# CMU-Perceptual-Computing-Lab/caffe_rtpose

Measured on AMD Instinct MI355X. Metric: frames/sec (whole node) at 656x368 COCO model, higher is better.
Workload: dtype f16; 1 GPU; COCO 656x368, 1 scale(s), synthetic 720p video: pageable host u8 1280x720 frames through rtp_submit_frame: pinned copy + H2D + device warp / INTER_AREA / normalise / pad inside the timed region -> conv stack+ImResize+NMS+connect -> joints on the host; precision mode mixed, 7 frames in flight/GPU in ; precision=mixed, input=host_u8, batch_frames=2, frames_in_flight=7, num_scales=1, exec=graph, hw_queues=4, parallelism=frame-sharded replicas x1

## Files before the change

### caffe_rtpose_amd/csrc/conv_pw2.hip

```cpp
#include "conv_common.h"
#include <atomic>
#include <type_traits>

namespace rtp {

namespace {
constexpr int PW_BM = 64;
constexpr int PW_ROW = 256;
constexpr int PW_STR = PW_ROW + 16;
constexpr int PW_X = PW_BM * PW_STR;
constexpr int PW_W = 128 * PW_STR;
constexpr int PW_MAXMID = 512;
constexpr int PW_LDS = 4 * PW_X + PW_W + PW_MAXMID * 4;
static_assert(PW_LDS >= 64 * 64 * 4, "epilogue scratch fits");
}

typedef unsigned int u32x32 __attribute__((ext_vector_type(32)));
typedef unsigned int u32x16 __attribute__((ext_vector_type(16)));
template <typename V>
__device__ __forceinline__ void pw_fetch(V& reg, const unsigned char* src, int tid) {
  constexpr int NV = sizeof(V) / 16;
#pragma unroll
  for (int i = 0; i < NV; ++i) {
    const uint4 t = *(const uint4*)(src + (size_t)(tid + i * 256) * 16);
    reg[4 * i] = t.x; reg[4 * i + 1] = t.y; reg[4 * i + 2] = t.z; reg[4 * i + 3] = t.w;
  }
}
template <typename V>
__device__ __forceinline__ void pw_stash(const V& reg, unsigned char* sW, int tid) {
  constexpr int NV = sizeof(V) / 16;
#pragma unroll
  for (int i = 0; i < NV; ++i) {
    const int v = tid + i * 256;
    uint4 t;
    t.x = reg[4 * i]; t.y = reg[4 * i + 1]; t.z = reg[4 * i + 2]; t.w = reg[4 * i + 3];
    *(uint4*)(sW + (v >> 4) * PW_STR + (v & 15) * 16) = t;
  }
}

__global__ __launch_bounds__(256) void conv_pw2_kernel(Pw2Params Q) {
  const KStamp kstamp_(Q.P2.stamp);
  extern __shared__ __attribute__((aligned(16))) unsigned char smem[];
  unsigned char* sXh = smem;
  unsigned char* sXl = smem + PW_X;
  unsigned char* sHh = smem + 2 * PW_X;
  unsigned char* sHl = smem + 3 * PW_X;
  unsigned char* sW = smem + 4 * PW_X;
  float* sB1 = (float*)(smem + 4 * PW_X + PW_W);

  const ConvParams& P = Q.P2;
  const int tid = threadIdx.x, lane = tid & 63, wave = tid >> 6;
  const int lrow = lane & 31, lhalf = lane >> 5;
  const int total_m = P.tiles_per_img * P.nimg;
  const int prob = blockIdx.x / total_m;
  const int mt = blockIdx.x % total_m;
  const int img = mt / P.tiles_per_img;
  const int m0 = (mt % P.tiles_per_img) * PW_BM;
  const ConvProblem& pr = P.prob[prob];
  const long pix0 = (long)img * P.img_pix + (long)P.halo * P.Wp + m0;
  const int Mtot = P.H * P.Wp;
  int stamp_i = 0;
  auto stamp = [&]() __attribute__((always_inline)) {
    if (P.clkprobe && blockIdx.x == 0 && tid == 0 && stamp_i < 31) P.clkprobe[1 + stamp_i++] = wall_clock64();
  };
  stamp();

  const float* b1p = prob ? Q.b1[1] : Q.b1[0];
  const int nmid = Q.c1_chunks * 128;
  const float b_a = tid < nmid ? b1p[tid] : 0.f;
  const float b_b = tid + 256 < nmid ? b1p[tid + 256] : 0.f;
  u32x16 r_xh, r_xl;
  {
    const _Float16* xin = (const _Float16*)(prob ? Q.x_in[1] : Q.x_in[0]) + pix0 * Q.x_cstride;
#pragma unroll
    for (int i = 0; i < 4; ++i) {
      const int v = tid + i * 256, row = v >> 4, seg = v & 15;
      const unsigned char* src = (const unsigned char*)(xin + (long)row * Q.x_cstride) + seg * 16;
      const uint4 h = *(const uint4*)src;
      r_xh[4 * i] = h.x; r_xh[4 * i + 1] = h.y; r_xh[4 * i + 2] = h.z; r_xh[4 * i + 3] = h.w;
      if (Q.x_lo_off) {
        const uint4 l = *(const uint4*)(src + (size_t)Q.x_lo_off * 2);
        r_xl[4 * i] = l.x; r_xl[4 * i + 1] = l.y; r_xl[4 * i + 2] = l.z; r_xl[4 * i + 3] = l.w;
      }
    }
  }
  u32x32 r_w1h, r_w1l;
  u32x16 r_w2h, r_w2l;
  auto lds_barrier = [&]() __attribute__((always_inline)) { asm volatile("s_waitcnt lgkmcnt(0)\n\ts_barrier" ::: "memory"); };
  auto gemm = [&](const unsigned char* a_img, int a_row0, auto ntm_tag, int b_row0, floatx16* acc) __attribute__((always_inline)) {
    constexpr int NT = decltype(ntm_tag)::value;
    const unsigned char* pb = sW + (b_row0 + lrow) * PW_STR + lhalf * 16;
    const unsigned char* pa = a_img + (a_row0 + lrow) * PW_STR + lhalf * 16;
#pragma unroll
    for (int g = 0; g < 8; ++g) {
      const uint4 fb = *(const uint4*)(pb + g * 32);
#pragma unroll
      for (int i = 0; i < NT; ++i) {
        const uint4 fa = *(const uint4*)(pa + i * 32 * PW_STR + g * 32);
        Mma<_Float16>::run(fa, fb, acc[i]);
      }
    }
  };
  const std::integral_constant<int, 2> two{};
  const std::integral_constant<int, 1> one{};

  const int w1_parts = Q.split_w1 ? 2 : 1, w2_parts = Q.split_w2 ? 2 : 1;
  const unsigned char* w1 = (const unsigned char*)(prob ? Q.w1[1] : Q.w1[0]);
  const unsigned char* w2 = (const unsigned char*)(prob ? P.prob[1].w : P.prob[0].w);
  const size_t W1_BLK = 128 * PW_ROW, W2_BLK = 64 * PW_ROW;
  auto w1_blk = [&](int c, int part) { return w1 + ((size_t)c * w1_parts + part) * W1_BLK; };
  auto w2_blk = [&](int c, int part) { return w2 + ((size_t)c * w2_parts + part) * W2_BLK; };

  floatx16 acc2;
#pragma unroll
  for (int q = 0; q < 16; ++q) acc2[q] = 0.f;

  pw_fetch(r_w1h, w1_blk(0, 0), tid);
  if (Q.split_w1) pw_fetch(r_w1l, w1_blk(0, 1), tid);
  pw_fetch(r_w2h, w2_blk(0, 0), tid);
  if (Q.split_w2) pw_fetch(r_w2l, w2_blk(0, 1), tid);
  sB1[tid] = b_a;
  sB1[tid + 256] = b_b;
#pragma unroll
  for (int i = 0; i < 4; ++i) {
    const int v = tid + i * 256, row = v >> 4, seg = v & 15;
    uint4 t;
    t.x = r_xh[4 * i]; t.y = r_xh[4 * i + 1]; t.z = r_xh[4 * i + 2]; t.w = r_xh[4 * i + 3];
    *(uint4*)(sXh + row * PW_STR + seg * 16) = t;
    if (Q.x_lo_off) {
      t.x = r_xl[4 * i]; t.y = r_xl[4 * i + 1]; t.z = r_xl[4 * i + 2]; t.w = r_xl[4 * i + 3];
      *(uint4*)(sXl + row * PW_STR + seg * 16) = t;
    }
  }
  stamp();
  for (int c = 0; c < Q.c1_chunks; ++c) {
    const bool more = c + 1 < Q.c1_chunks;
    floatx16 acc1[2];
#pragma unroll
    for (int i = 0; i < 2; ++i)
#pragma unroll
      for (int q = 0; q < 16; ++q) acc1[i][q] = 0.f;
    lds_barrier();
    pw_stash(r_w1h, sW, tid);
    if (more) pw_fetch(r_w1h, w1_blk(c + 1, 0), tid);
    lds_barrier();
    stamp();
    gemm(sXh, 0, two, wave * 32, acc1);
    if (Q.x_lo_off) gemm(sXl, 0, two, wave * 32, acc1);
    stamp();
    if (Q.split_w1) {
      lds_barrier();
      pw_stash(r_w1l, sW, tid);
      if (more) pw_fetch(r_w1l, w1_blk(c + 1, 1), tid);
      lds_barrier();
      gemm(sXh, 0, two, wave * 32, acc1);
      stamp();
    }
    {
      const float bias = sB1[c * 128 + wave * 32 + lrow];
#pragma unroll
      for (int i = 0; i < 2; ++i)
#pragma unroll
        for (int q = 0; q < 16; ++q) {
          const int row = i * 32 + (q & 3) + 8 * (q >> 2) + 4 * lhalf;
          float v = acc1[i][q] + bias;
          if (Q.relu1) v = v > 0.f ? v : 0.f;
          const _Float16 hi = (_Float16)v;
          *(_Float16*)(sHh + row * PW_STR + (wave * 32 + lrow) * 2) = hi;
          if (Q.h_lo) *(_Float16*)(sHl + row * PW_STR + (wave * 32 + lrow) * 2) = (_Float16)(v - (float)hi);
        }
    }
    stamp();
    lds_barrier();
    pw_stash(r_w2h, sW, tid);
    if (more) pw_fetch(r_w2h, w2_blk(c + 1, 0), tid);
    lds_barrier();
    stamp();
    gemm(sHh, (wave >> 1) * 32, one, (wave & 1) * 32, &acc2);
    if (Q.h_lo) gemm(sHl, (wave >> 1) * 32, one, (wave & 1) * 32, &acc2);
    stamp();
    const ConvDst& md = prob ? Q.mid[1] : Q.mid[0];
    if (md.base) {
      for (int v = tid; v < PW_BM * 16; v += 256) {
        const int row = v >> 4, seg = v & 15;
        const int m = m0 + row;
        const int xp = m - (m / P.Wp) * P.Wp;
        if (m >= Mtot || xp < P.halo || xp >= P.halo + P.W) continue;
        _Float16* dp = (_Float16*)md.base + (pix0 + row) * md.cstride + md.coff + c * 128 + seg * 8;
        *(uint4*)dp = *(const uint4*)(sHh + row * PW_STR + seg * 16);
        if (md.lo_off) *(uint4*)(dp + md.lo_off) = *(const uint4*)(sHl + row * PW_STR + seg * 16);
      }
    }
    stamp();
    if (Q.split_w2) {
      lds_barrier();
      pw_stash(r_w2l, sW, tid);
      if (more) pw_fetch(r_w2l, w2_blk(c + 1, 1), tid);
      lds_barrier();
      gemm(sHh, (wave >> 1) * 32, one, (wave & 1) * 32, &acc2);
      stamp();
    }
  }
  __syncthreads();
  stamp();
  floatx16 acc[1][1] = {{acc2}};
  conv_epilogue<_Float16, 64, 64, 2, 2, 1, 1, 1>(P, pr, acc, smem, 0, wave, (wave >> 1) * 32, (wave & 1) * 32, lane, img, m0, 0);
  stamp();
  if (P.clkprobe && blockIdx.x == 0 && tid == 0) P.clkprobe[0] = stamp_i;
}

hipError_t launch_conv_pw2(const Pw2Params& Q, int nprob, int nimg, hipStream_t stream) {
  static std::atomic<unsigned> attr_mask{0};
  int dev = 0;
  (void)hipGetDevice(&dev);
  if (!(attr_mask.load(std::memory_order_relaxed) & (1u << (dev & 31)))) {
    hipError_t e = hipFuncSetAttribute((const void*)conv_pw2_kernel, hipFuncAttributeMaxDynamicSharedMemorySize, PW_LDS);
    if (e != hipSuccess) return e;
    attr_mask.fetch_or(1u << (dev & 31), std::memory_order_relaxed);
  }
  dim3 grid(Q.P2.tiles_per_img * nimg * nprob);
  hipLaunchKernelGGL(conv_pw2_kernel, grid, dim3(256), PW_LDS, stream, Q);
  return hipGetLastError();
}

}
```

### caffe_rtpose_amd/csrc/engine.cpp

```cpp
#include <hip/hip_runtime.h>

#include <algorithm>
#include <atomic>
#include <chrono>
#include <cmath>
#include <cstdarg>
#include <cstdio>
#include <cstring>
#include <deque>
#include <fstream>
#include <map>
#include <mutex>
#include <sstream>
#include <string>
#include <thread>
#include <vector>

#include "../../include/rtpose_mi355x.h"
#include "kernels.h"
#include "netdef.h"
#include "plan.h"

using namespace rtp;

// ... 195 lines not shown
  }
  const int M = (int)std::nearbyint(std::ldexp(a, 9));
  return (unsigned char)(sign | (unsigned)(M == 8 ? 8 : M));
}

template <typename T>
void pack_conv(const Plan& plan, const ConvOp& c, const std::vector<float>& w, const std::vector<float>& b,
               std::vector<unsigned char>* out_w, std::vector<float>* out_b) {
  const Tensor& ti = plan.tensors[c.in_tensor];
  const int per_chunk = c.rowb / (int)sizeof(T);
  const int taps = c.k_eff * c.k_eff;
  out_w->assign(c.w_bytes, 0);
  T* pw = (T*)out_w->data();
  auto kpos = [&](int n, int kk) {
    if (c.impl == 0) return kk;
    const int per16 = 16 / (int)sizeof(T);
    const int c16 = kk / per16, within = kk % per16;
    return ((c16 ^ conv_ring_swz(c.rowb, n)) * per16) + within;
  };
  if (c.direct_first) {
    for (int t = 0; t < 2; ++t)
      for (int j = 0; j < 2; ++j)
        for (int l = 0; l < 64; ++l) {
          const int n = t * 32 + conv_first_channel_of_row(l & 31);
          for (int e2 = 0; e2 < 8; ++e2) {
            const int k = j * 16 + (l >> 5) * 8 + e2;
            float wv = 0.f;
            if (k < 27) { const int r = k / 9, s2 = (k % 9) / 3, cc = k % 3; wv = w[((size_t)(n * 3 + cc) * 3 + r) * 3 + s2]; }
            pw[((size_t)(t * 2 + j) * 64 + l) * 8 + e2] = (T)wv;
          }
        }
    out_b->assign(c.CoutP, 0.f);
    for (int n = 0; n < c.cout; ++n) (*out_b)[n] = b[n];
    return;
  }
  if (c.fused) {
    const int rows = c.fused == 1 ? 128 : 64;
    const int parts = c.split_w ? 2 : 1;
    for (int n = 0; n < c.cout; ++n)
      for (int cr = 0; cr < c.cin; ++cr) {
        const int ci = ti.chmap[cr];
        const int chunk = c.fused == 1 ? n / 128 : ci / 128;
        const int row = c.fused == 1 ? n % 128 : n;
        const int k = ci % 128;
        const float wv = w[(size_t)n * c.cin + cr];
        const T hi = (T)wv;
        pw[(((size_t)chunk * parts + 0) * rows + row) * 128 + k] = hi;
        if (c.split_w) pw[(((size_t)chunk * parts + 1) * rows + row) * 128 + k] = (T)(wv - (float)hi);
      }
    out_b->assign(c.CoutP, 0.f);
    for (int n = 0; n < c.cout; ++n) (*out_b)[n] = b[n];
    return;
  }
  if (c.first) {
    for (int n = 0; n < c.cout; ++n)
      for (int r = 0; r < 3; ++r)
        for (int s = 0; s < 3; ++s)
          for (int cc = 0; cc < 3; ++cc) {
            const int j = (r * 3 + s) * 3 + cc;
            const int chunk = j / per_chunk, kk = j % per_chunk;
            const float wv = w[((size_t)(n * 3 + cc) * 3 + r) * 3 + s];
            const T hi = (T)wv;
            pw[((size_t)(0 * c.nchunk + chunk) * c.CoutP + n) * per_chunk + kpos(n, kk)] = hi;
            if (c.split_w) pw[((size_t)(0 * c.nchunk + c.ncp + chunk) * c.CoutP + n) * per_chunk + kpos(n, kk)] = (T)(wv - (float)hi);
          }
  } else {
    for (int n = 0; n < c.cout; ++n)
      for (int cr = 0; cr < c.cin; ++cr) {
        const int ci = ti.chmap[cr];
        const int chunk = ci / per_chunk, kk = ci % per_chunk;
        for (int r = 0; r < c.k; ++r)
          for (int s = 0; s < c.k; ++s) {
            const int tap = r * c.k + s;
            const float wv = w[((size_t)(n * c.cin + cr) * c.k + r) * c.k + s];
            const T hi = (T)wv;
            const T lo = (T)(wv - (float)hi);
            if (c.h8) {
              const size_t tile0 = (size_t)(r * c.nchunk + chunk) * c.k + s;
              pw[(tile0 * c.CoutP + n) * per_chunk + kpos(n, kk)] = hi;
              const size_t tileq = (size_t)(r * c.nchunk + c.ncp + chunk) * c.k + s;
              unsigned char* qrow = out_w->data() + (tileq * c.CoutP + n) * c.rowb;
              const int g = kk / 64, pos = kk % 64;
              auto qpos = [&](int byte) { return ((byte / 16) ^ conv_ring_swz(c.rowb, n)) * 16 + byte % 16; };
              qrow[qpos(g * 128 + pos)] = f32_to_e4m3(std::ldexp((float)hi, c.wq_exp));
              qrow[qpos(g * 128 + 64 + pos)] = f32_to_e4m3(std::ldexp(wv - (float)hi, c.wq_exp + 11));
              continue;
            }
            int vbase = 0;
            for (int pass = 0; pass < 3; ++pass) {
              if ((pass == 1 && !c.split_a) || (pass == 2 && !c.split_w)) continue;
              const int vchunk = vbase + chunk;
              vbase += c.ncp;
              const size_t tile = c.impl == 1 ? ((size_t)(r * c.nchunk + vchunk) * c.k + s) : ((size_t)tap * c.nchunk + vchunk);
              pw[(tile * c.CoutP + n) * per_chunk + kpos(n, kk)] = pass == 2 ? lo : hi;
            }
          }
      }
  }
  out_b->assign(c.CoutP, 0.f);
  for (int n = 0; n < c.cout; ++n) (*out_b)[n] = b[n];
}

void compute_wq_exp(rtp_engine* e) {
  for (auto& s : e->plan.steps) {
    if (s.type != 1 || !e->plan.convs[s.a].h8) continue;
    float mx = 0.f;
    for (int idx : {s.a, s.b}) if (idx >= 0) for (float v : e->w_ref[idx]) mx = std::max(mx, std::fabs(v));
    int ex = mx > 0.f ? (int)std::floor(std::log2(448.0 / mx)) : 0;
    ex = std::max(-20, std::min(ex, 40));
    for (int idx : {s.a, s.b}) if (idx >= 0) e->plan.convs[idx].wq_exp = ex;
  }
}

int upload_conv_weights(rtp_engine* e, int i) {
  const ConvOp& c = e->plan.convs[i];
  std::vector<unsigned char> pw;
  std::vector<float> pb;
  if (e->plan.prec == 0) pack_conv<_Float16>(e->plan, c, e->w_ref[i], e->b_ref[i], &pw, &pb);
  else pack_conv<float>(e->plan, c, e->w_ref[i], e->b_ref[i], &pw, &pb);
  SYNC_GUARD;
  HIPCHK(e, hipMemcpy(e->dweights + c.w_off, pw.data(), pw.size(), hipMemcpyHostToDevice));
  HIPCHK(e, hipMemcpy(e->dweights + c.b_off, pb.data(), pb.size() * sizeof(float), hipMemcpyHostToDevice));
  return RTP_OK;
}

int upload_all_weights(rtp_engine* e) {
  std::vector<unsigned char> image(e->plan.weights_bytes, 0);
  const int n = (int)e->plan.convs.size();
  const int nthr = std::max(1, std::min({(int)std::thread::hardware_concurrency(), 16, n}));
  std::atomic<int> next{0};
  auto work = [&]() {
    std::vector<unsigned char> pw;
    std::vector<float> pb;
    for (int i = next.fetch_add(1); i < n; i = next.fetch_add(1)) {
      const ConvOp& c = e->plan.convs[i];
      if (e->plan.prec == 0) pack_conv<_Float16>(e->plan, c, e->w_ref[i], e->b_ref[i], &pw, &pb);
      else pack_conv<float>(e->plan, c, e->w_ref[i], e->b_ref[i], &pw, &pb);
      memcpy(image.data() + c.w_off, pw.data(), pw.size());
      memcpy(image.data() + c.b_off, pb.data(), pb.size() * sizeof(float));
    }
  };
  std::vector<std::thread> pool;
  for (int t = 1; t < nthr; ++t) pool.emplace_back(work);
  work();
  for (auto& t : pool) t.join();
  SYNC_GUARD;
  HIPCHK(e, hipMemcpy(e->dweights, image.data(), e->plan.weights_bytes, hipMemcpyHostToDevice));
  return RTP_OK;
}

constexpr int STAMP_SLOTS = 256;
unsigned long long* stamp_slot(const rtp_engine* e, const Ctx& cx, int idx) {
  return (e->stamp_probe && cx.stamps && idx >= 0 && idx < STAMP_SLOTS) ? cx.stamps + 2 * (size_t)idx : nullptr;
}
int stamp_harvest(rtp_engine* e, Ctx& cx) {
  if (!cx.stamps || !cx.stamps_dirty) return RTP_OK;
  for (Slot& sl : cx.slot)
    if (sl.export_pending) HIPCHK(e, hipEventSynchronize(sl.ev_export));
  std::vector<unsigned long long> h(2 * STAMP_SLOTS);
  HIPCHK(e, hipMemcpy(h.data(), cx.stamps, h.size() * sizeof(unsigned long long), hipMemcpyDeviceToHost));
  HIPCHK(e, hipMemset(cx.stamps, 0, h.size() * sizeof(unsigned long long)));
  cx.stamps_dirty = false;
  for (int i = 0; i < STAMP_SLOTS; ++i) {
    if (!h[2 * i + 1] || !h[2 * i]) continue;
    const unsigned long long t0 = ~h[2 * i], t1 = h[2 * i + 1];
    if (!e->stamp_base) e->stamp_base = t0;
    if (e->stamp_spans.size() < 3 * (size_t)(1 << 20)) {
      e->stamp_spans.push_back((float)i);
      e->stamp_spans.push_back((float)((double)((long long)(t0 - e->stamp_base)) * 0.01));
      e->stamp_spans.push_back((float)((double)((long long)(t1 - e->stamp_base)) * 0.01));
    }
  }
  return RTP_OK;
}

void fill_problem(const rtp_engine* e, const Ctx& cx, const ConvOp& c, ConvProblem* pr) {
  memset(pr, 0, sizeof(*pr));
  pr->in = cx.arena + e->plan.tensors[c.in_tensor].offset;
  pr->w = e->dweights + c.w_off;
  pr->bias = (const float*)(e->dweights + c.b_off);
  pr->ndst = (int)c.dsts.size();
  for (int d = 0; d < pr->ndst; ++d) {
    const Tensor& t = e->plan.tensors[c.dsts[d].first];
    pr->dst[d].base = cx.arena + t.offset;
    pr->dst[d].cstride = t.stride();
    pr->dst[d].coff = c.dsts[d].second;
    pr->dst[d].lo_off = t.lo_off();
    pr->dst[d].q_off = t.q_off();
  }
  if (c.to_lowres) {
    pr->out_nchw = cx.lowres;
    pr->out_C = e->plan.heat_channels;
    pr->out_coff = c.lowres_coff;
  }
  pr->Cout = c.cout;
}

unsigned long long* g_clkprobe = nullptr;
int launch_conv_step(rtp_engine* e, Ctx& cx, const Step& s, int nimg) {
  const ConvOp& A = e->plan.convs[s.a];
  const Geom& g = e->plan.geom[A.level];
  ConvParams P;
  memset(&P, 0, sizeof P);
  fill_problem(e, cx, A, &P.prob[0]);
  if (s.b >= 0) fill_problem(e, cx, e->plan.convs[s.b], &P.prob[1]);
  P.H = g.H; P.W = g.W; P.Wp = g.Wp; P.halo = g.halo; P.img_pix = g.img_pix;
  P.in_cstride = e->plan.tensors[A.in_tensor].stride();
  P.nchunk = A.nchunk;
  P.wrap_at = A.wrap_at();
  P.last_phys = A.last_phys();
  {
    const Tensor& tin = e->plan.tensors[A.in_tensor];
    const int qb = tin.q_off() * e->plan.elem;
    P.q_from = A.h8 ? A.ncp : 0;
    P.jump_delta = A.h8 ? qb - (A.ncp - 1) * A.rowb : 0;
    P.row_back = A.h8 ? qb + (A.ncp - 1) * A.rowb : A.last_phys() * A.rowb;
    P.wq_exp = A.wq_exp;
  }
  P.CoutP = A.CoutP;
  P.tiles_per_img = (int)conv_tiles_per_img(e->plan, A);
  if (A.pool >= 0) {
    const Geom& go = e->plan.geom[A.level + 1];
    P.pool = 1;
    P.pool_wq = pool_wq(g, A);
    P.pool_Wp = go.Wp; P.pool_halo = go.halo; P.pool_img_pix = go.img_pix;
  }
  P.relu = A.relu ? 1 : 0;
  P.clkprobe = g_clkprobe;
  P.stamp = stamp_slot(e, cx, (int)(&s - e->plan.steps.data()));
  P.nimg = nimg;
  {
    static const char* rot = RTP_EXP_ENV("RTP_CONV_ROTATE");
    P.rotate = (rot && rot[0] == '0') ? 0 : 1;
    static const char* xm = RTP_EXP_ENV("RTP_CONV_XCDMAP");
    P.xcdmap = xm ? atoi(xm) : 1;
    static const char* sb = RTP_EXP_ENV("RTP_RING_SB");
    P.ring_sb = sb ? atoi(sb) : 6;
    static const char* sp = RTP_EXP_ENV("RTP_RING_SPEC");
    P.spec = (sp && sp[0] == '0') ? 0 : 1;
    static const char* rv = RTP_EXP_ENV("RTP_RING_VAR");
    P.variant = rv ? atoi(rv) : 0;
    static const char* ed = RTP_EXP_ENV("RTP_EPI_DIAG");
    P.diag = ed ? atoi(ed) : 0;
    static const char* il = RTP_EXP_ENV("RTP_RING_ILV");
    P.ilv = il ? (il[0] == '1' || (il[0] == 'q' && A.h8) || (il[0] == '7' && A.h8 && A.k_eff == 7)) : (A.h8 ? 1 : 0);
  }
  if (A.impl == 1) HIPCHK(e, launch_conv_ring(e->plan.prec, A.cfg, A.k_eff, A.rowb, P, s.b >= 0 ? 2 : 1, nimg, cx.stream));
  else HIPCHK(e, launch_conv(e->plan.prec, A.cfg, A.k_eff, A.rowb, P, s.b >= 0 ? 2 : 1, nimg, cx.stream));
  return RTP_OK;
}

int launch_pw2_step(rtp_engine* e, Ctx& cx, const Step& s, int nimg) {
  const ConvOp& A = e->plan.convs[s.a];
  const ConvOp& C = e->plan.convs[s.a2];
  const Geom& g = e->plan.geom[C.level];
  Pw2Params Q;
  memset(&Q, 0, sizeof Q);
  ConvParams& P = Q.P2;
  fill_problem(e, cx, C, &P.prob[0]);
  if (s.b2 >= 0) fill_problem(e, cx, e->plan.convs[s.b2], &P.prob[1]);
  P.H = g.H; P.W = g.W; P.Wp = g.Wp; P.halo = g.halo; P.img_pix = g.img_pix;
  P.CoutP = 64;
  P.tiles_per_img = (int)plain_tiles_per_img(g, 64);
  P.relu = C.relu ? 1 : 0;
  P.stamp = stamp_slot(e, cx, (int)(&s - e->plan.steps.data()));
  P.nimg = nimg;
  const int firsts[2] = {s.a, s.b};
  for (int q = 0; q < 2; ++q) {
    if (firsts[q] < 0) continue;
    const ConvOp& F = e->plan.convs[firsts[q]];
    const Tensor& ti = e->plan.tensors[F.in_tensor];
    const Tensor& tm = e->plan.tensors[F.dsts[0].first];
    Q.x_in[q] = cx.arena + ti.offset;
    Q.x_cstride = ti.stride();
    Q.x_lo_off = F.split_a ? ti.lo_off() : 0;
    Q.w1[q] = e->dweights + F.w_off;
    Q.b1[q] = (const float*)(e->dweights + F.b_off);
    Q.mid[q].base = tm.written ? cx.arena + tm.offset : nullptr;
    Q.mid[q].cstride = tm.stride();
    Q.mid[q].coff = 0;
    Q.mid[q].lo_off = tm.lo_off();
  }
  Q.c1_chunks = A.fused_chunks;
  Q.relu1 = A.relu ? 1 : 0;
  Q.split_w1 = A.split_w ? 1 : 0;
  Q.split_w2 = C.split_w ? 1 : 0;
  Q.h_lo = C.split_a ? 1 : 0;
  static const char* probe = RTP_EXP_ENV("RTP_PW2_PROBE");
  static int probed = 0;
  hipStreamCaptureStatus cst = hipStreamCaptureStatusNone;
  if (probe) (void)hipStreamIsCapturing(cx.stream, &cst);
  if (probe && cst == hipStreamCaptureStatusNone && probed < 16) {
    unsigned long long* d = nullptr;
    HIPCHK(e, hipMalloc((void**)&d, 32 * 8));
    HIPCHK(e, hipMemset(d, 0, 32 * 8));
    P.clkprobe = d;
    const auto t0 = std::chrono::steady_clock::now();
    HIPCHK(e, launch_conv_pw2(Q, s.b >= 0 ? 2 : 1, nimg, cx.stream));
    HIPCHK(e, hipStreamSynchronize(cx.stream));
    const double host_us = std::chrono::duration<double, std::micro>(std::chrono::steady_clock::now() - t0).count();
    unsigned long long h[32];
    HIPCHK(e, hipMemcpy(h, d, sizeof h, hipMemcpyDeviceToHost));
    (void)hipFree(d);
    fprintf(stderr, "pw2 probe %s chunks %d splits %d%d%d%d (launch+sync %.1f us): ", A.name.c_str(), Q.c1_chunks, Q.x_lo_off ? 1 : 0, Q.split_w1, Q.h_lo, Q.split_w2, host_us);
    for (unsigned i = 2; i <= h[0] && i < 32; ++i) fprintf(stderr, "%.2f ", (double)(h[i] - h[i - 1]) / 100.0);
    fprintf(stderr, "us; total %.2f us\n", (double)(h[h[0]] - h[1]) / 100.0);
    ++probed;
    return RTP_OK;
  }
  HIPCHK(e, launch_conv_pw2(Q, s.b >= 0 ? 2 : 1, nimg, cx.stream));
  return RTP_OK;
}

}

namespace {
bool is_dominant_class(const rtp_engine* e, const Step& s) {
  if (s.type != 1 || e->plan.dominant_step < 0) return false;
  const ConvOp& a = e->plan.convs[s.a];
  const ConvOp& d = e->plan.convs[e->plan.steps[e->plan.dominant_step].a];
  return a.k == d.k && a.cin == d.cin && a.cout == d.cout && (s.b >= 0) == (e->plan.steps[e->plan.dominant_step].b >= 0);
}

int launch_first_step(rtp_engine* e, Ctx& cx, const Step& s, const float* input_dev, int nimg) {
  const ConvOp& c = e->plan.convs[s.a];
  const Tensor& to = e->plan.tensors[c.dsts[0].first];
  FirstParams Q;
  Q.in = input_dev;
  Q.g = e->plan.geom[0];
  Q.g.N = nimg;
  Q.wfrag = (const uint4*)(e->dweights + c.w_off);
  Q.bias = (const float*)(e->dweights + c.b_off);
  Q.out = (_Float16*)(cx.arena + to.offset);
  Q.Cp = to.stride();
  Q.relu = c.relu ? 1 : 0;
  Q.stamp = stamp_slot(e, cx, (int)(&s - e->plan.steps.data()));
  HIPCHK(e, launch_conv_first(Q, cx.stream));
  return RTP_OK;
}

int run_frame_stack(rtp_engine* e, Ctx& cx, const float* input_dev, int nimg, bool cap = false) {
  const std::vector<PoolOp>& pools = e->plan.pools;
  auto geom_n = [&](int level) { Geom g = e->plan.geom[level]; g.N = nimg; return g; };
  for (size_t si = 0; si < e->plan.steps.size(); ++si) {
    const Step& s = e->plan.steps[si];
    const bool want_timed = e->time_dominant && !cap && nimg == e->plan.NI && (e->time_all || is_dominant_class(e, s));
    const bool timed = want_timed && e->tev_next < (int)e->tev.size() / 2;
    if (want_timed && !timed) e->probe_dropped[0]++;
    if (timed) HIPCHK(e, hipEventRecord(e->tev[2 * (size_t)e->tev_next], cx.stream));
    struct Close {
      rtp_engine* e; Ctx& cx; const Step& s; size_t si; bool timed;
      ~Close() {
        if (!timed) return;
        (void)hipEventRecord(e->tev[2 * (size_t)e->tev_next + 1], cx.stream);
        e->tev_step[e->tev_next] = (short)si;
        e->tev_pass[e->tev_next++] = (unsigned char)(s.type == 1 ? e->plan.convs[s.a].passes() : 1);
      }
    } close_{e, cx, s, si, timed};
    if (s.type == 0) {
      const Tensor& t = e->plan.tensors[0];
      HIPCHK(e, launch_pack_input(e->plan.prec, input_dev, cx.arena + t.offset, geom_n(0), t.stride(), cx.stream));
    } else if (s.type == 1) {
      const int rc = launch_conv_step(e, cx, s, nimg);
      if (rc) return rc;
    } else if (s.type == 3) {
      const int rc = launch_pw2_step(e, cx, s, nimg);
      if (rc) return rc;
    } else if (s.type == 4) {
      const int rc = launch_first_step(e, cx, s, input_dev, nimg);
      if (rc) return rc;
    } else {
      const PoolOp& p = pools[s.a];
      const Tensor& ti = e->plan.tensors[p.in_tensor];
      const Tensor& to = e->plan.tensors[p.out_tensor];
      HIPCHK(e, launch_maxpool(e->plan.prec, cx.arena + ti.offset, geom_n(ti.level), ti.stride(), cx.arena + to.offset, geom_n(to.level), to.stride(),
                               round_up(p.C, 16 / e->plan.elem), ti.lo_off(), to.lo_off(), ti.q_off(), to.q_off(), cx.stream));
    }
  }
  return RTP_OK;
}

ResizeParams resize_params(rtp_engine* e, Ctx& cx, int sj) {
  Slot& sl = cx.slot[sj];
  ResizeParams rp;
  rp.src = cx.lowres + (size_t)sj * e->N * e->plan.heat_channels * e->plan.low_h * e->plan.low_w;
  rp.dst = sl.resized; rp.num = e->N; rp.C = e->plan.heat_channels;
  rp.h = e->plan.low_h; rp.w = e->plan.low_w; rp.tw = e->cfg.net_w; rp.th = e->cfg.net_h;
  rp.start_scale = e->start_scale; rp.scale_gap = e->scale_gap;
  return rp;
}
int run_resize(rtp_engine* e, Ctx& cx, int sj = 0) {
  HIPCHK(e, launch_resize(resize_params(e, cx, sj), cx.slot[sj].stream));
  return RTP_OK;
}
NmsParams nms_params(rtp_engine* e, Ctx& cx, int sj) {
  Slot& sl = cx.slot[sj];
  NmsParams np;
  np.src = sl.resized; np.peaks = sl.peaks; np.strip_count = sl.strip_count; np.strip_list = sl.strip_list;
  np.src_planes = e->plan.heat_channels; np.H = e->cfg.net_h; np.W = e->cfg.net_w; np.num_parts = e->plan.num_parts;
  np.max_peaks = e->plan.max_peaks; np.nstrips = e->plan.nstrips; np.strip_rows = e->plan.strip_rows; np.threshold = e->nms_threshold;
  np.probe = nullptr;
  np.clear_flag = nullptr;
  np.stamp = stamp_slot(e, cx, 64 + 8 * sj);
  return np;
}
int run_nms(rtp_engine* e, Ctx& cx, int sj = 0) {
  HIPCHK(e, launch_nms(nms_params(e, cx, sj), cx.slot[sj].stream));
  return RTP_OK;
}
ConnectParams connect_params(rtp_engine* e, Ctx& cx, int sj) {
  Slot& sl = cx.slot[sj];
  ConnectParams cp;
  memset(&cp, 0, sizeof cp);
  cp.heat = sl.resized; cp.peaks = sl.peaks; cp.joints = sl.joints; cp.num_people = sl.num_people;
  cp.cand_score = sl.cand_score; cp.cand_ij = sl.cand_ij; cp.cand_count = sl.cand_count; cp.cand_blk = sl.cand_blk;
  cp.conn = sl.conn; cp.conn_score = sl.conn_score; cp.conn_count = sl.conn_count;
  cp.max_rows = e->plan.max_rows; cp.model = e->plan.model; cp.num_parts = e->plan.num_parts; cp.num_limbs = e->plan.num_limbs;
  cp.max_peaks = e->plan.max_peaks; cp.net_w = e->cfg.net_w; cp.net_h = e->cfg.net_h; cp.disp_w = e->cfg.disp_w; cp.disp_h = e->cfg.disp_h;
  cp.inter_threshold = e->inter_threshold; cp.inter_min_above = e->inter_min_above; cp.min_subset_cnt = e->min_subset_cnt;
  cp.min_subset_score = e->min_subset_score; cp.max_people = RTP_MAX_PEOPLE;
  cp.stamp = stamp_slot(e, cx, 64 + 8 * sj + 2);
  {
    static const char* pf = RTP_EXP_ENV("RTP_PAIRS_FULL");
    cp.pairs_full = (pf && pf[0] == '1') ? 1 : 0;
  }
  return cp;
}
int run_connect(rtp_engine* e, Ctx& cx, int sj = 0) {
  HIPCHK(e, launch_connect(connect_params(e, cx, sj), cx.slot[sj].stream));
  return RTP_OK;
}
int run_post_fused(rtp_engine* e, Ctx& cx, int sj, hipEvent_t ev_nms) {
  Slot& sl = cx.slot[sj];
  const ResizeParams rp = resize_params(e, cx, sj);
  NmsParams np = nms_params(e, cx, sj);
  np.clear_flag = sl.num_people;
  HIPCHK(e, launch_nms_fused(np, rp, sl.stream));
  HIPCHK(e, hipEventRecord(ev_nms, sl.stream));
  ConnectParams cp = connect_params(e, cx, sj);
  cp.counter_cleared = 1;
  cp.tickets = e->chain_connect ? sl.tickets : nullptr;
  HIPCHK(e, launch_connect_fused(cp, rp, sl.stream));
  return RTP_OK;
}

int jpeg_alloc(rtp_engine* e, int w, int h, JpegBufs* b, unsigned char** host, unsigned char** host_dev, size_t* cap);

int launch_batch_body(rtp_engine* e, Ctx& cx, int nframes, const float* input_dev, bool materialize, bool cap, int part = 3) {
  int rc;
  if (part & 1) {
    HIPCHK(e, hipEventRecord(cx.ev[0], cx.stream));
    if ((rc = run_frame_stack(e, cx, input_dev, nframes * e->N, cap))) return rc;
  }
  if (!(part & 2)) return RTP_OK;
  HIPCHK(e, hipEventRecord(cx.ev[1], cx.stream));
  const size_t jbytes = (size_t)RTP_MAX_PEOPLE * e->plan.num_parts * 3 * sizeof(float);
  for (int j = 0; j < nframes; ++j) {
    Slot& sl = cx.slot[j];
    if (sl.stream != cx.stream) HIPCHK(e, hipStreamWaitEvent(sl.stream, cx.ev[1], 0));
    static const char* diag = RTP_EXP_ENV("RTP_DIAG_SKIP_POST");
    const int skip = diag ? atoi(diag) : 0;
    static const char* unf = RTP_EXP_ENV("RTP_POST_UNFUSED");
    HIPCHK(e, hipEventRecord(sl.ev[0], sl.stream));
    if (skip >= 3) {
      const ResizeParams rp = resize_params(e, cx, j);
      HIPCHK(e, hipEventRecord(sl.ev[1], sl.stream));
      HIPCHK(e, launch_nms_fused(nms_params(e, cx, j), rp, sl.stream));
      HIPCHK(e, hipEventRecord(sl.ev[2], sl.stream));
      if (skip >= 4) {
        ConnectParams cp = connect_params(e, cx, j);
        cp.diag_stages = skip - 3;
        HIPCHK(e, launch_connect_fused(cp, rp, sl.stream));
      }
    } else if (materialize || skip || (unf && unf[0] == '1')) {
      if (skip < 2 && (rc = run_resize(e, cx, j))) return rc;
      HIPCHK(e, hipEventRecord(sl.ev[1], sl.stream));
      if (skip < 2 && (rc = run_nms(e, cx, j))) return rc;
      HIPCHK(e, hipEventRecord(sl.ev[2], sl.stream));
      if (skip < 1 && (rc = run_connect(e, cx, j))) return rc;
    } else {
      HIPCHK(e, hipEventRecord(sl.ev[1], sl.stream));
      if ((rc = run_post_fused(e, cx, j, sl.ev[2]))) return rc;
    }
    HIPCHK(e, hipEventRecord(sl.ev[3], sl.stream));
    if (e->cfg.render && sl.has_disp) {
      const size_t dbytes = (size_t)e->cfg.disp_w * e->cfg.disp_h * 3;
      if (!sl.render_dev) {
        SYNC_GUARD;
        HIPCHK(e, hipMalloc((void**)&sl.render_dev, dbytes));
        HIPCHK(e, hipHostMalloc((void**)&sl.render_host, dbytes, hipHostMallocDefault));
        HIPCHK(e, hipMalloc((void**)&sl.render_tab, render_tab_floats(RTP_MAX_PEOPLE) * sizeof(float)));
      }
      if (e->cfg.render == 1) {
        RenderParams rp;
        rp.src = sl.disp_cur; rp.dst = sl.render_dev; rp.w = e->cfg.disp_w; rp.h = e->cfg.disp_h;
        rp.poses = sl.joints; rp.num_people = sl.num_people; rp.tab = sl.render_tab;
        rp.model = e->plan.model; rp.googly = 0; rp.max_people = RTP_MAX_PEOPLE;
        HIPCHK(e, launch_render(rp, sl.stream));
      } else {
        if (!(materialize || skip || (unf && unf[0] == '1')) && (rc = run_resize(e, cx, j))) return rc;
        RenderViewParams vp;
        vp.src = sl.disp_cur; vp.dst = sl.render_dev; vp.w = e->cfg.disp_w; vp.h = e->cfg.disp_h;
        vp.maps = sl.resized; vp.net_w = e->cfg.net_w; vp.net_h = e->cfg.net_h;
        vp.model = e->plan.model; vp.part_to_show = e->cfg.render - 1;
        HIPCHK(e, launch_render_view(vp, sl.stream));
      }
      if (e->jpeg_quality) {
        if (!sl.jpeg.base) {
          SYNC_GUARD;
          if ((rc = jpeg_alloc(e, e->cfg.disp_w, e->cfg.disp_h, &sl.jpeg, &sl.jpeg_host, &sl.jpeg_host_dev, &sl.jpeg_cap))) return rc;
        }
        const FrameView fv = {sl.render_dev, e->cfg.disp_w, e->cfg.disp_h, 3L * e->cfg.disp_w, 3L, {0L, 1L, 2L}};
        HIPCHK(e, launch_jpeg_encode(stamp_slot(e, cx, 64 + 8 * j + 6), fv, e->jpeg_q, sl.jpeg, sl.jpeg_host_dev,
                                     reinterpret_cast<unsigned*>(sl.jpeg_host_dev + sl.jpeg_cap), sl.stream));
      } else {
        if (!sl.render_host) {
          SYNC_GUARD;
          HIPCHK(e, hipHostMalloc((void**)&sl.render_host, dbytes, hipHostMallocDefault));
        }
        HIPCHK(e, hipMemcpyAsync(sl.render_host, sl.render_dev, dbytes, hipMemcpyDeviceToHost, sl.stream));
      }
    }
    HIPCHK(e, hipMemcpyAsync(sl.host_out + 4, sl.joints, jbytes, hipMemcpyDeviceToHost, sl.stream));
    HIPCHK(e, hipMemcpyAsync(sl.host_out, sl.num_people, sizeof(int), hipMemcpyDeviceToHost, sl.stream));
    HIPCHK(e, hipEventRecord(sl.ev[4], sl.stream));
    if (cap && sl.stream != cx.stream) HIPCHK(e, hipStreamWaitEvent(cx.stream, sl.ev[4], 0));
  }
  return RTP_OK;
}

int capture_batch(rtp_engine* e, Ctx& cx, int nframes, hipGraphExec_t* out) {
  SYNC_GUARD;
  hipGraph_t g = nullptr;
  HIPCHK(e, hipStreamBeginCapture(cx.stream, hipStreamCaptureModeThreadLocal));
  const int rc = launch_batch_body(e, cx, nframes, cx.input, false, true, e->graph_post ? 3 : 1);
  const hipError_t s = hipStreamEndCapture(cx.stream, &g);
  if (rc) { if (g) (void)hipGraphDestroy(g); return rc; }
  if (s != hipSuccess || !g) return fail(e, RTP_EHIP, "hipStreamEndCapture failed: %s", hipGetErrorString(s));
  const hipError_t si = hipGraphInstantiate(out, g, nullptr, nullptr, 0);
  (void)hipGraphDestroy(g);
  if (si != hipSuccess) return fail(e, RTP_EHIP, "hipGraphInstantiate failed: %s", hipGetErrorString(si));
  return RTP_OK;
}

int flush_prep(rtp_engine* e, Ctx& cx, bool force);
int launch_batch(rtp_engine* e, Ctx& cx, int nframes, const float* input_dev, bool materialize = false) {
  int rc;
  for (Slot& sl : cx.slot)
    if (sl.export_pending) {
      HIPCHK(e, hipStreamWaitEvent(cx.stream, sl.ev_export, 0));
      sl.export_pending = false;
    }
  if (e->prep_defer && (rc = flush_prep(e, cx, true))) return rc;
  if (cx.in_pending) {
    if (cx.in_stream != cx.stream) {
      HIPCHK(e, hipEventRecord(cx.ev_in, cx.in_stream));
      HIPCHK(e, hipStreamWaitEvent(cx.stream, cx.ev_in, 0));
    }
    cx.in_pending = false;
  }
  static const char* diag = RTP_EXP_ENV("RTP_DIAG_SKIP_POST");
  static const char* unf = RTP_EXP_ENV("RTP_POST_UNFUSED");
  const bool graph = e->use_graph && !e->time_dominant && !materialize && input_dev == cx.input && !e->cfg.render && !diag && !unf && nframes <= 16;
  cx.graph_run = graph;
  cx.graph_conv = false;
  if (!graph) {
    if ((rc = launch_batch_body(e, cx, nframes, input_dev, materialize, false))) return rc;
    cx.launched = true;
    return RTP_OK;
  }
  if (!cx.gexec[nframes] && (rc = capture_batch(e, cx, nframes, &cx.gexec[nframes]))) return rc;
  HIPCHK(e, hipEventRecord(cx.gev[0], cx.stream));
  HIPCHK(e, hipGraphLaunch(cx.gexec[nframes], cx.stream));
  if (!e->graph_post) {
    if ((rc = launch_batch_body(e, cx, nframes, cx.input, false, false, 2))) return rc;
    cx.graph_run = false;
    cx.graph_conv = true;
  }
  HIPCHK(e, hipEventRecord(cx.gev[1], cx.stream));
  cx.launched = true;
  return RTP_OK;
}
int enqueue_frame(rtp_engine* e, Ctx& cx, const float* input_dev, bool materialize = false) { return launch_batch(e, cx, 1, input_dev, materialize); }

int hw_queue_count() {
  const char* v = getenv("GPU_MAX_HW_QUEUES");
  const int q = v ? atoi(v) : 4;
  return q >= 1 && q <= 64 ? q : 4;
}
hipError_t make_stream(hipStream_t* s, bool post) {
#ifdef RTP_EXPERIMENTS
  if (post) {
    const char* c = getenv("RTP_POST_CUS");
    const int n = c ? atoi(c) : 0;
    if (n > 0 && n < 256) {
      uint32_t mask[8] = {0, 0, 0, 0, 0, 0, 0, 0};
      for (int b = 0; b < n; ++b) mask[b >> 5] |= 1u << (b & 31);
      return hipExtStreamCreateWithCUMask(s, 8, mask);
    }
  }
  const char* v = getenv(post ? "RTP_POST_PRIO" : "RTP_CONV_PRIO");
  if (v && v[0]) {
    int least = 0, greatest = 0;
    (void)hipDeviceGetStreamPriorityRange(&least, &greatest);
    int pr = atoi(v);
    pr = std::max(greatest, std::min(least, pr));
    return hipStreamCreateWithPriority(s, hipStreamNonBlocking, pr);
// ... 2276 lines not shown
```

### caffe_rtpose_amd/csrc/kernels.h

```cpp
#pragma once
#include <hip/hip_runtime.h>
#include <stdint.h>
#include <stdlib.h>

#include "jpeg_bound.h"

#ifdef RTP_EXPERIMENTS
#define RTP_EXP_ENV(name) getenv(name)
#else
#define RTP_EXP_ENV(name) ((const char*)nullptr)
#endif

namespace rtp {

#if defined(__HIPCC__)
struct KStamp {
  unsigned long long* s;
  __device__ __forceinline__ explicit KStamp(unsigned long long* p) : s(p) {
    if (s && threadIdx.x == 0 && threadIdx.y == 0) atomicMax(s, ~wall_clock64());
  }
  __device__ __forceinline__ ~KStamp() {
    if (s && threadIdx.x == 0 && threadIdx.y == 0) atomicMax(s + 1, wall_clock64());
  }
};
#endif

struct Geom {
  int N, H, W, halo, Hp, Wp;
  long img_pix;
};

#define RTP_MAX_DST 6
struct ConvDst {
  void* base;
  int cstride;
  int coff;
  int lo_off;
  int q_off;
};

struct ConvProblem {
  const void* in;
  const void* w;
  const float* bias;
  ConvDst dst[RTP_MAX_DST];
  int ndst;
  float* out_nchw;
  int out_C, out_coff;
  int Cout;
};

struct ConvParams {
  ConvProblem prob[2];
  int H, W, Wp, halo;
  long img_pix;
  int in_cstride;
  int nchunk;
  int wrap_at;
  int last_phys;
  int q_from;
  int wq_exp;
  int jump_delta;
  int row_back;
  int CoutP;
  int tiles_per_img;
  int nimg;
  int relu;
  int rotate;
  int xcdmap;
  int ring_sb;
  int spec;
  int variant;
  int ilv;
  int pool, pool_wq, pool_Wp, pool_halo;
  long pool_img_pix;
  int diag;
  unsigned long long* stamp;
  unsigned long long* clkprobe;
};

enum ConvCfg { CFG_128x128 = 0, CFG_64x128 = 1, CFG_64x64 = 2, CFG_128x64 = 3, CFG_128x32 = 4, CFG_256x64 = 5, CFG_COUNT = 6 };

struct ConvCfgInfo { int BM, BN; };
inline ConvCfgInfo conv_cfg_info(int cfg) {
  switch (cfg) {
    case CFG_128x128: return {128, 128};
    case CFG_64x128: return {64, 128};
    case CFG_64x64: return {64, 64};
    case CFG_128x32: return {128, 32};
    case CFG_256x64: return {256, 64};
    default: return {128, 64};
  }
}

hipError_t launch_conv(int prec, int cfg, int ks, int rowb, const ConvParams& P, int nprob, int N,
                       hipStream_t stream);

hipError_t launch_conv_ring(int prec, int cfg, int ks, int chb, const ConvParams& P, int nprob, int N,
                            hipStream_t stream);
struct Pw2Params {
  ConvParams P2;
  const void* x_in[2];
  int x_cstride, x_lo_off;
  const void* w1[2];
  const float* b1[2];
  ConvDst mid[2];
  int c1_chunks;
  int relu1;
  int split_w1, split_w2, h_lo;
};
hipError_t launch_conv_pw2(const Pw2Params& Q, int nprob, int nimg, hipStream_t stream);

inline int conv_ring_swz(int chb, int row) { return chb == 256 ? (row & 15) : ((row >> 1) & 7); }

hipError_t launch_pack_input(int prec, const float* in_nchw, void* out, Geom g, int Cp, hipStream_t stream);
struct FirstParams {
  const float* in;
  Geom g;
  const uint4* wfrag;
  const float* bias;
  _Float16* out;
  int Cp;
  int relu;
  unsigned long long* stamp;
};
hipError_t launch_conv_first(const FirstParams& Q, hipStream_t stream);
int conv_first_channel_of_row(int i);
hipError_t launch_maxpool(int prec, const void* in, Geom gi, int Cpi, void* out, Geom go, int Cpo, int C, int lo_i, int lo_o, int q_i, int q_o,
                          hipStream_t stream);
hipError_t launch_export(int prec, const void* in, Geom g, int Cp, const int* chmap_dev, int C, int lo_off, int q_off, float* out,
                         hipStream_t stream);

struct AreaScale {
  int tw, th, identity;
  int fast_x, fast_y;
  const int* xstart; const int* xsi; const float* xalpha;
  const int* ystart; const int* ysi; const float* yalpha;
  int linear;
  const int* lx; const int* ly;
};
hipError_t launch_warp(unsigned long long* stamp, const unsigned char* src, int sw, int sh, double inv, const short* tab2d, unsigned char* dst, int dw, int dh,
                       hipStream_t stream);
hipError_t launch_area_pad(unsigned long long* stamp, const unsigned char* disp, int dw, int dh, const AreaScale* scales, int nscales, float* out, int net_w, int net_h,
                           hipStream_t stream);

struct FrameView {
  unsigned char* data;
  int w, h;
  long row, pix;
  long off[3];
};
enum FrameLayout { LAYOUT_GENERIC = 0, LAYOUT_HWC3_BGR, LAYOUT_HWC3_RGB, LAYOUT_HWC4_BGR, LAYOUT_HWC4_RGB, LAYOUT_PLANAR };
int frame_layout(const FrameView& v, size_t avail);
hipError_t launch_frame_import(unsigned long long* stamp, const FrameView& v, int layout, unsigned char* dst, hipStream_t stream);
hipError_t launch_frame_export(unsigned long long* stamp, const unsigned char* src, const FrameView& v, int layout, hipStream_t stream);
hipError_t launch_warp_view(unsigned long long* stamp, const FrameView& v, double inv, const short* tab2d, unsigned char* dst, int dw, int dh,
                            hipStream_t stream);

struct YuvView {
  const unsigned char* y;
  const unsigned char* u;
  const unsigned char* v;
  int w, h, sx, sy;
  long ys, uvs, uvp;
};
enum YuvLayout { YUV_GENERIC = 0, YUV_420_PLANAR, YUV_420_NV12, YUV_420_NV21 };
int yuv_layout(const YuvView& s, const FrameView& d);
inline FrameView packed_bgr_view(unsigned char* p, int w, int h) { return FrameView{p, w, h, 3L * w, 3, {0, 1, 2}}; }
hipError_t launch_yuv_import(unsigned long long* stamp, const YuvView& s, const FrameView& d, int layout, hipStream_t stream);

struct JpegHuffTab { unsigned short code[256]; unsigned char size[256]; };
struct JpegQuant { unsigned recip[2][64]; unsigned short half[2][64]; };
struct JpegBufs {
  void* base = nullptr;
  int w = 0, h = 0;
  JpegHuffTab* huff = nullptr;
  short* coef = nullptr;
  unsigned* bits = nullptr;
  unsigned* mcubits = nullptr;
  unsigned* off = nullptr;
  int* dcdiff = nullptr;
  unsigned* words = nullptr;
  unsigned* counts = nullptr;
  unsigned* meta = nullptr;
  unsigned char* data = nullptr;
};
size_t jpeg_bufs_bytes(int w, int h, JpegBufs* layout);
hipError_t launch_jpeg_encode(unsigned long long* stamp, const FrameView& v, const JpegQuant& q, const JpegBufs& jb, unsigned char* dst,
                              unsigned* dst_len, hipStream_t stream);

struct RenderParams {
  const unsigned char* src;
  unsigned char* dst;
  int w, h;
  const float* poses;
  const int* num_people;
  float* tab;
  int model, googly, max_people;
};
hipError_t launch_render(const RenderParams& p, hipStream_t stream);
size_t render_tab_floats(int max_people);
struct RenderViewParams {
  const unsigned char* src;
  unsigned char* dst;
  int w, h;
  const float* maps;
  int net_w, net_h;
  int model, part_to_show;
};
hipError_t launch_render_view(const RenderViewParams& p, hipStream_t stream);

struct ResizeParams {
  const float* src;
  float* dst;
  int num, C, h, w, tw, th;
  float start_scale, scale_gap;
};
hipError_t launch_resize(const ResizeParams& p, hipStream_t stream);

struct NmsParams {
  const float* src;
  float* peaks;
  int* strip_count;
  int* strip_list;
  int src_planes, H, W, num_parts, max_peaks, nstrips, strip_rows;
  float threshold;
  unsigned long long* probe;
  unsigned long long* stamp;
  int* clear_flag;
};
hipError_t launch_nms(const NmsParams& p, hipStream_t stream);
hipError_t launch_nms_fused(const NmsParams& p, const ResizeParams& r, hipStream_t stream);

struct ConnectParams {
  unsigned long long* stamp;
  int counter_cleared;
  int* tickets;
  const float* heat;
  const float* peaks;
  float* joints;
  int* num_people;
  float* cand_score;
  int* cand_ij;
  int* cand_count;
  int* cand_blk;
  int* conn;
  float* conn_score;
  int* conn_count;
  int* subset_idx;
  double* subset_score;
  int* subset_cnt;
  int max_rows;
  int assemble_preload;
  int pairs_full;
  int diag_stages;
  int model;
  int num_parts, num_limbs, max_peaks;
  int net_w, net_h, disp_w, disp_h;
  float inter_threshold;
  int inter_min_above;
  int min_subset_cnt;
  float min_subset_score;
  int max_people;
};
hipError_t launch_connect(const ConnectParams& p, hipStream_t stream);
hipError_t launch_connect_fused(const ConnectParams& p, const ResizeParams& r, hipStream_t stream);

}
```

Before: 1060 frames/s.

## Alias pw2 LDS buffers for single-chunk case to fit two workgroups per CU

For the fused pointwise-pair conv kernel, when only one mid-channel chunk exists, the hidden-activation LDS buffers now alias the input buffers. This shrinks LDS so two workgroups fit per CU, and launch bounds now request 2 blocks. The first GEMM swaps its MFMA operand order so the intermediate can be written with vectorised 4-wide stores and bias loaded as float4. An extra barrier is added before the aliased write, and the tighter register budget from the launch bound may cause spills. The old path is kept behind an experiment flag.

```diff
diff --git a/caffe_rtpose_amd/csrc/conv_pw2.hip b/caffe_rtpose_amd/csrc/conv_pw2.hip
--- a/caffe_rtpose_amd/csrc/conv_pw2.hip
+++ b/caffe_rtpose_amd/csrc/conv_pw2.hip
@@ -12,7 +12,9 @@
 constexpr int PW_W = 128 * PW_STR;
 constexpr int PW_MAXMID = 512;
 constexpr int PW_LDS = 4 * PW_X + PW_W + PW_MAXMID * 4;
-static_assert(PW_LDS >= 64 * 64 * 4, "epilogue scratch fits");
+constexpr int PW_LDS1 = 2 * PW_X + PW_W + PW_MAXMID * 4;
+static_assert(PW_LDS >= 64 * 64 * 4 && PW_LDS1 >= 64 * 64 * 4, "epilogue scratch fits");
+static_assert(2 * PW_LDS1 <= 160 * 1024, "two single-chunk workgroups per CU");
 }
 
 typedef unsigned int u32x32 __attribute__((ext_vector_type(32)));
@@ -38,15 +40,16 @@
   }
 }
 
-__global__ __launch_bounds__(256) void conv_pw2_kernel(Pw2Params Q) {
+template <bool LEGACY>
+__device__ __forceinline__ void conv_pw2_body(const Pw2Params& Q, unsigned char* smem) {
   const KStamp kstamp_(Q.P2.stamp);
-  extern __shared__ __attribute__((aligned(16))) unsigned char smem[];
+  const bool alias = !LEGACY && Q.c1_chunks == 1;
   unsigned char* sXh = smem;
   unsigned char* sXl = smem + PW_X;
-  unsigned char* sHh = smem + 2 * PW_X;
-  unsigned char* sHl = smem + 3 * PW_X;
-  unsigned char* sW = smem + 4 * PW_X;
-  float* sB1 = (float*)(smem + 4 * PW_X + PW_W);
+  unsigned char* sHh = alias ? sXh : smem + 2 * PW_X;
+  unsigned char* sHl = alias ? sXl : smem + 3 * PW_X;
+  unsigned char* sW = smem + (alias ? 2 : 4) * PW_X;
+  float* sB1 = (float*)(sW + PW_W);
 
   const ConvParams& P = Q.P2;
   const int tid = threadIdx.x, lane = tid & 63, wave = tid >> 6;
@@ -87,8 +90,9 @@
   u32x32 r_w1h, r_w1l;
   u32x16 r_w2h, r_w2l;
   auto lds_barrier = [&]() __attribute__((always_inline)) { asm volatile("s_waitcnt lgkmcnt(0)\n\ts_barrier" ::: "memory"); };
-  auto gemm = [&](const unsigned char* a_img, int a_row0, auto ntm_tag, int b_row0, floatx16* acc) __attribute__((always_inline)) {
+  auto gemm = [&](const unsigned char* a_img, int a_row0, auto ntm_tag, int b_row0, floatx16* acc, auto swap_tag) __attribute__((always_inline)) {
     constexpr int NT = decltype(ntm_tag)::value;
+    constexpr bool SWAP = decltype(swap_tag)::value;
     const unsigned char* pb = sW + (b_row0 + lrow) * PW_STR + lhalf * 16;
     const unsigned char* pa = a_img + (a_row0 + lrow) * PW_STR + lhalf * 16;
 #pragma unroll
@@ -97,12 +101,15 @@
 #pragma unroll
       for (int i = 0; i < NT; ++i) {
         const uint4 fa = *(const uint4*)(pa + i * 32 * PW_STR + g * 32);
-        Mma<_Float16>::run(fa, fb, acc[i]);
+        if constexpr (SWAP) Mma<_Float16>::run(fb, fa, acc[i]);
+        else Mma<_Float16>::run(fa, fb, acc[i]);
       }
     }
   };
   const std::integral_constant<int, 2> two{};
   const std::integral_constant<int, 1> one{};
+  const std::integral_constant<bool, !LEGACY> sw1{};
+  const std::integral_constant<bool, false> nosw{};
 
   const int w1_parts = Q.split_w1 ? 2 : 1, w2_parts = Q.split_w2 ? 2 : 1;
   const unsigned char* w1 = (const unsigned char*)(prob ? Q.w1[1] : Q.w1[0]);
@@ -145,18 +152,40 @@
     if (more) pw_fetch(r_w1h, w1_blk(c + 1, 0), tid);
     lds_barrier();
     stamp();
-    gemm(sXh, 0, two, wave * 32, acc1);
-    if (Q.x_lo_off) gemm(sXl, 0, two, wave * 32, acc1);
+    gemm(sXh, 0, two, wave * 32, acc1, sw1);
+    if (Q.x_lo_off) gemm(sXl, 0, two, wave * 32, acc1, sw1);
     stamp();
     if (Q.split_w1) {
       lds_barrier();
       pw_stash(r_w1l, sW, tid);
       if (more) pw_fetch(r_w1l, w1_blk(c + 1, 1), tid);
       lds_barrier();
-      gemm(sXh, 0, two, wave * 32, acc1);
+      gemm(sXh, 0, two, wave * 32, acc1, sw1);
       stamp();
     }
-    {
+    if constexpr (!LEGACY) lds_barrier();
+    if constexpr (!LEGACY) {
+#pragma unroll
+      for (int g = 0; g < 4; ++g) {
+        const int ch = wave * 32 + 8 * g + 4 * lhalf;
+        const float4 bias = *(const float4*)(sB1 + c * 128 + ch);
+        const float bs[4] = {bias.x, bias.y, bias.z, bias.w};
+#pragma unroll
+        for (int i = 0; i < 2; ++i) {
+          _Float16 hi[4], lo[4];
+#pragma unroll
+          for (int u = 0; u < 4; ++u) {
+            float v = acc1[i][4 * g + u] + bs[u];
+            if (Q.relu1) v = v > 0.f ? v : 0.f;
+            hi[u] = (_Float16)v;
+            lo[u] = (_Float16)(v - (float)hi[u]);
+          }
+          const int off = (i * 32 + lrow) * PW_STR + ch * 2;
+          *(uint2*)(sHh + off) = __builtin_bit_cast(uint2, hi);
+          if (Q.h_lo) *(uint2*)(sHl + off) = __builtin_bit_cast(uint2, lo);
+        }
+      }
+    } else {
       const float bias = sB1[c * 128 + wave * 32 + lrow];
 #pragma unroll
       for (int i = 0; i < 2; ++i)
@@ -171,13 +200,13 @@
         }
     }
     stamp();
-    lds_barrier();
+    if constexpr (LEGACY) lds_barrier();
     pw_stash(r_w2h, sW, tid);
     if (more) pw_fetch(r_w2h, w2_blk(c + 1, 0), tid);
     lds_barrier();
     stamp();
-    gemm(sHh, (wave >> 1) * 32, one, (wave & 1) * 32, &acc2);
-    if (Q.h_lo) gemm(sHl, (wave >> 1) * 32, one, (wave & 1) * 32, &acc2);
+    gemm(sHh, (wave >> 1) * 32, one, (wave & 1) * 32, &acc2, nosw);
+    if (Q.h_lo) gemm(sHl, (wave >> 1) * 32, one, (wave & 1) * 32, &acc2, nosw);
     stamp();
     const ConvDst& md = prob ? Q.mid[1] : Q.mid[0];
     if (md.base) {
@@ -197,7 +226,7 @@
       pw_stash(r_w2l, sW, tid);
       if (more) pw_fetch(r_w2l, w2_blk(c + 1, 1), tid);
       lds_barrier();
-      gemm(sHh, (wave >> 1) * 32, one, (wave & 1) * 32, &acc2);
+      gemm(sHh, (wave >> 1) * 32, one, (wave & 1) * 32, &acc2, nosw);
       stamp();
     }
   }
@@ -207,6 +236,36 @@
   conv_epilogue<_Float16, 64, 64, 2, 2, 1, 1, 1>(P, pr, acc, smem, 0, wave, (wave >> 1) * 32, (wave & 1) * 32, lane, img, m0, 0);
   stamp();
   if (P.clkprobe && blockIdx.x == 0 && tid == 0) P.clkprobe[0] = stamp_i;
+}
+
+__global__ __launch_bounds__(256, 2) void conv_pw2_kernel(Pw2Params Q) {
+  extern __shared__ __attribute__((aligned(16))) unsigned char smem[];
+  conv_pw2_body<false>(Q, smem);
+}
+#ifdef RTP_EXPERIMENTS
+__global__ __launch_bounds__(256) void conv_pw2_kernel_legacy(Pw2Params Q) {
+  extern __shared__ __attribute__((aligned(16))) unsigned char smem[];
+  conv_pw2_body<true>(Q, smem);
+}
+#endif
+
+namespace {
+typedef void (*Pw2Kernel)(Pw2Params);
+Pw2Kernel pw2_select(const Pw2Params& Q, int* lds) {
+#ifdef RTP_EXPERIMENTS
+  static const char* legacy = RTP_EXP_ENV("RTP_PW2_LEGACY");
+  if (legacy && legacy[0] == '1') { *lds = PW_LDS; return conv_pw2_kernel_legacy; }
+#endif
+  *lds = Q.c1_chunks == 1 ? PW_LDS1 : PW_LDS;
+  return conv_pw2_kernel;
+}
+}
+
+int conv_pw2_blocks_per_cu(const Pw2Params& Q) {
+  int lds = 0, n = -1;
+  const Pw2Kernel k = pw2_select(Q, &lds);
+  if (hipOccupancyMaxActiveBlocksPerMultiprocessor(&n, (const void*)k, 256, (size_t)lds) != hipSuccess) return -1;
+  return n;
 }
 
 hipError_t launch_conv_pw2(const Pw2Params& Q, int nprob, int nimg, hipStream_t stream) {
@@ -216,10 +275,16 @@
   if (!(attr_mask.load(std::memory_order_relaxed) & (1u << (dev & 31)))) {
     hipError_t e = hipFuncSetAttribute((const void*)conv_pw2_kernel, hipFuncAttributeMaxDynamicSharedMemorySize, PW_LDS);
     if (e != hipSuccess) return e;
+#ifdef RTP_EXPERIMENTS
+    e = hipFuncSetAttribute((const void*)conv_pw2_kernel_legacy, hipFuncAttributeMaxDynamicSharedMemorySize, PW_LDS);
+    if (e != hipSuccess) return e;
+#endif
     attr_mask.fetch_or(1u << (dev & 31), std::memory_order_relaxed);
   }
+  int lds = 0;
+  const Pw2Kernel k = pw2_select(Q, &lds);
   dim3 grid(Q.P2.tiles_per_img * nimg * nprob);
-  hipLaunchKernelGGL(conv_pw2_kernel, grid, dim3(256), PW_LDS, stream, Q);
+  hipLaunchKernelGGL(k, grid, dim3(256), lds, stream, Q);
   return hipGetLastError();
 }
 
diff --git a/caffe_rtpose_amd/csrc/engine.cpp b/caffe_rtpose_amd/csrc/engine.cpp
--- a/caffe_rtpose_amd/csrc/engine.cpp
+++ b/caffe_rtpose_amd/csrc/engine.cpp
@@ -521,7 +521,8 @@
     unsigned long long h[32];
     HIPCHK(e, hipMemcpy(h, d, sizeof h, hipMemcpyDeviceToHost));
     (void)hipFree(d);
-    fprintf(stderr, "pw2 probe %s chunks %d splits %d%d%d%d (launch+sync %.1f us): ", A.name.c_str(), Q.c1_chunks, Q.x_lo_off ? 1 : 0, Q.split_w1, Q.h_lo, Q.split_w2, host_us);
+    fprintf(stderr, "pw2 probe %s chunks %d splits %d%d%d%d blocks/CU %d (launch+sync %.1f us): ", A.name.c_str(), Q.c1_chunks, Q.x_lo_off ? 1 : 0, Q.split_w1, Q.h_lo, Q.split_w2,
+            conv_pw2_blocks_per_cu(Q), host_us);
     for (unsigned i = 2; i <= h[0] && i < 32; ++i) fprintf(stderr, "%.2f ", (double)(h[i] - h[i - 1]) / 100.0);
     fprintf(stderr, "us; total %.2f us\n", (double)(h[h[0]] - h[1]) / 100.0);
     ++probed;
diff --git a/caffe_rtpose_amd/csrc/kernels.h b/caffe_rtpose_amd/csrc/kernels.h
--- a/caffe_rtpose_amd/csrc/kernels.h
+++ b/caffe_rtpose_amd/csrc/kernels.h
@@ -110,6 +110,7 @@
   int split_w1, split_w2, h_lo;
 };
 hipError_t launch_conv_pw2(const Pw2Params& Q, int nprob, int nimg, hipStream_t stream);
+int conv_pw2_blocks_per_cu(const Pw2Params& Q);
 
 inline int conv_ring_swz(int chb, int row) { return chb == 256 ? (row & 15) : ((row >> 1) & 7); }
 
```

Measured after the change: 1077 frames/s (median of 6 runs). 1.02x the previous value.
